# xswang/xflow

Measured on NVIDIA H100. Metric: training examples/sec, higher is better.
Workload: dtype f32

## Files before the change

xflow_b200/csrc/checkpoint.cu:

```cuda
#include <cuda_runtime.h>
#include <stddef.h>
#include <stdint.h>
#include <stdio.h>
#include <string.h>

#include <algorithm>
#include <string>
#include <vector>

#include "internal.h"

#define XF_ST_TILE 1024
#define XF_ST_VERSION 1u

struct XfStateHeader {
  char magic[4];
  uint32_t version;
  uint64_t header_bytes;
  uint64_t capacity;
  uint64_t cap_floor;
  uint64_t n_keys;
  uint32_t stride;
  uint32_t log2cap;
  uint32_t bshift;
  uint32_t lazy;
  int32_t latent_dim;
  int32_t optimizer;
  float alpha, beta, lambda1, lambda2, learning_rate;
  int32_t v_init;
  uint64_t seed;
  int32_t shard_index;
  int32_t num_shards;
  int32_t canonical_fm;
  uint32_t seq;
  uint64_t batches;
  uint64_t rejected_tokens;
  uint64_t admitted_keys;
  int32_t admit_mode;
  float admit_probability;
  uint32_t admit_threshold;
  uint32_t admit_log2_cells;
  uint32_t admit_hashes;
  uint32_t tracking;
  uint64_t admit_decay_batches;
  uint64_t admit_seed;
  uint64_t evict_max_idle_batches;
// ... 147 lines not shown
  if (lane == 0) atomicAdd(meta_out + 1, sum);
  if (blockIdx.x == 0 && threadIdx.x == 0) meta_out[0] = total;
}

__global__ void __launch_bounds__(256) xf_k_state_unpack(XfTableView t, uint32_t* __restrict__ stamp,
                                                         const uint8_t* __restrict__ in, uint64_t n, uint64_t first,
                                                         uint64_t chunk_slots, uint64_t tag,
                                                         unsigned long long* __restrict__ sum_out, int* __restrict__ bad) {
  const uint32_t q = t.stride / 16u;
  const uint64_t* meta = reinterpret_cast<const uint64_t*>(in + n * t.stride);
  const uint64_t items = n * q;
  unsigned long long sum = 0;
  for (uint64_t j = (uint64_t)blockIdx.x * blockDim.x + threadIdx.x; j < items; j += (uint64_t)gridDim.x * blockDim.x) {
    const uint64_t r = j / q;
    const uint32_t c16 = (uint32_t)(j - r * q);
    const uint64_t off = r * t.stride + 16u * c16;
    const uint4 v = *reinterpret_cast<const uint4*>(in + off);
    sum += xf_st_hash((uint64_t)v.x | ((uint64_t)v.y << 32), tag | off) +
           xf_st_hash((uint64_t)v.z | ((uint64_t)v.w << 32), tag | (off + 8));
    const uint64_t m = meta[r];
    if (c16 == 0) sum += xf_st_hash(m, tag | (n * t.stride + r * 8u));
    const uint64_t slot = (uint32_t)m;
    if (slot < first || slot >= first + chunk_slots || slot > t.mask) {
      if (c16 == 0) *bad = 1;
      continue;
    }
    *reinterpret_cast<uint4*>(xf_row(t, slot) + 16u * c16) = v;
    if (c16 == 0 && stamp != nullptr) stamp[slot] = (uint32_t)(m >> 32);
  }
  sum = xf_st_warp_sum(sum);
  if ((threadIdx.x & 31u) == 0) atomicAdd(sum_out, sum);
}

__global__ void __launch_bounds__(256) xf_k_state_sum(const uint64_t* __restrict__ p, uint64_t n_words, uint64_t off0,
                                                      unsigned long long* __restrict__ sum_out) {
  unsigned long long sum = 0;
  for (uint64_t i = (uint64_t)blockIdx.x * blockDim.x + threadIdx.x; i < n_words; i += (uint64_t)gridDim.x * blockDim.x)
    sum += xf_st_hash(p[i], off0 + i * 8u);
  sum = xf_st_warp_sum(sum);
  if ((threadIdx.x & 31u) == 0) atomicAdd(sum_out, sum);
}

static uint64_t xf_st_chunk_slots(uint32_t stride, uint64_t capacity) {
  uint64_t c = XF_ST_TILE;
  while (c * 2 <= capacity && c * 2 * (stride + 8ull) <= XF_ST_CHUNK_BYTES) c *= 2;
  return std::min(c, capacity);
}

struct XfStateIo {
  uint8_t* dev[2] = {nullptr, nullptr};
  uint8_t* pin[2] = {nullptr, nullptr};
  uint32_t* d_tiles[2] = {nullptr, nullptr};
  unsigned long long* d_small = nullptr;
  unsigned long long* h_small = nullptr;
  cudaStream_t copy = nullptr;
  cudaStream_t work = nullptr;
  cudaEvent_t done[2] = {nullptr, nullptr};
  cudaEvent_t copied[2] = {nullptr, nullptr};
  size_t bytes = 0;
  ~XfStateIo() {
    if (work) cudaStreamSynchronize(work);
    if (copy) cudaStreamSynchronize(copy);
    for (int b = 0; b < 2; ++b) {
      if (done[b]) cudaEventSynchronize(done[b]);
      if (dev[b]) cudaFree(dev[b]);
      if (pin[b]) cudaFreeHost(pin[b]);
// ... 95 lines not shown
    ++t->launches;
    XF_CUDA_TRY(cudaGetLastError());
    for (uint64_t j = 0; j < nf + 1; ++j) {
      if (j < nf) {
        const int b = (int)(j & 1);
        XF_CUDA_TRY(cudaMemcpyAsync(io.pin[b], t->d_filter + j * fc, fc, cudaMemcpyDeviceToHost, st));
        XF_CUDA_TRY(cudaEventRecord(io.copied[b], st));
      }
      if (j >= 1) {
        const int b = (int)((j - 1) & 1);
        XF_CUDA_TRY(cudaEventSynchronize(io.copied[b]));
        if (!xf_st_write(f, io.pin[b], fc)) { xf_set_error("write to %s failed", path); return XF_ERR_IO; }
      }
    }
    uint64_t s = 0;
    XF_CUDA_TRY(cudaMemcpyAsync(&s, io.d_small + 5, 8, cudaMemcpyDeviceToHost, st));
    XF_CUDA_TRY(cudaStreamSynchronize(st));
    if (!xf_st_write(f, &s, 8)) { xf_set_error("write to %s failed", path); return XF_ERR_IO; }
  }
  return XF_OK;
}

XF_DLL int xf_table_save_state(xf_table* t, const char* path, uint64_t user) {
  if (!t || !path) { xf_set_error("null argument"); return XF_ERR_ARG; }
  std::lock_guard<std::mutex> host_lock(t->host_mu);
  XF_CUDA_TRY(cudaSetDevice(t->cfg.device));
  XF_TRY(t->check_error());
  unsigned long long size = 0, counters[2] = {0ull, 0ull};
  XF_CUDA_TRY(cudaMemcpy(&size, t->d_size, sizeof(size), cudaMemcpyDeviceToHost));
  if (t->d_admit) XF_CUDA_TRY(cudaMemcpy(counters, t->d_admit, sizeof(counters), cudaMemcpyDeviceToHost));
  XfStateHeader h;
  memset(&h, 0, sizeof(h));
  memcpy(h.magic, "XFST", 4);
  h.version = XF_ST_VERSION;
  h.header_bytes = sizeof(h);
  h.capacity = t->view.mask + 1;
  h.cap_floor = t->cap_floor;
  h.n_keys = size;
  h.stride = t->view.stride;
  h.log2cap = t->view.log2cap;
  h.bshift = t->view.bshift;
  h.lazy = (uint32_t)t->view.lazy;
  h.latent_dim = t->cfg.latent_dim;
  h.optimizer = t->cfg.optimizer;
  h.alpha = t->cfg.alpha; h.beta = t->cfg.beta; h.lambda1 = t->cfg.lambda1; h.lambda2 = t->cfg.lambda2;
  h.learning_rate = t->cfg.learning_rate;
  h.v_init = t->view.v_init;
  h.seed = t->cfg.seed;
  h.shard_index = t->cfg.shard_index;
  h.num_shards = t->cfg.num_shards;
  h.canonical_fm = t->cfg.canonical_fm;
  h.seq = t->view.lazy ? t->seq : 0u;
  h.batches = t->admit_batches;
  h.rejected_tokens = counters[0];
  h.admitted_keys = counters[1];
  h.admit_mode = t->admit.mode;
  h.admit_probability = t->admit.probability;
  h.admit_threshold = t->admit.threshold;
  h.admit_log2_cells = t->admit.log2_cells;
  h.admit_hashes = t->admit.hashes;
  h.admit_decay_batches = t->admit.decay_batches;
  h.admit_seed = t->admit.seed;
  h.tracking = t->d_stamp != nullptr ? 1u : 0u;
  h.evict_max_idle_batches = t->evict.max_idle_batches;
  h.evict_max_keys = t->evict.max_keys;
  h.user = user;
  h.chunk_slots = xf_st_chunk_slots(h.stride, h.capacity);
// ... 130 lines not shown
    XF_CUDA_TRY(cudaEventRecord(io.done[b], st));
  }
  if (total != h.n_keys) { xf_set_error("state image %s: the rows section holds %llu rows, its header announces %llu", path, (unsigned long long)total, (unsigned long long)h.n_keys); return XF_ERR_IO; }
  uint64_t filter_stated = 0;
  if (h.filter_bytes) {
    const uint64_t fc = std::min<uint64_t>(h.filter_bytes, (uint64_t)1 << (63 - __builtin_clzll(io.bytes)));
    const uint64_t nf = h.filter_bytes / fc;
    for (uint64_t j = 0; j < nf; ++j) {
      const int b = (int)(j & 1);
      XF_CUDA_TRY(cudaEventSynchronize(io.copied[b]));
      if (!xf_st_read(f, io.pin[b], fc)) { xf_set_error("truncated state image %s", path); return XF_ERR_IO; }
      XF_CUDA_TRY(cudaMemcpyAsync(nw.filter + j * fc, io.pin[b], fc, cudaMemcpyHostToDevice, io.copy));
      XF_CUDA_TRY(cudaEventRecord(io.copied[b], io.copy));
    }
    if (!xf_st_read(f, &filter_stated, 8)) { xf_set_error("truncated state image %s", path); return XF_ERR_IO; }
    XF_CUDA_TRY(cudaEventRecord(io.done[0], io.copy));
    XF_CUDA_TRY(cudaStreamWaitEvent(st, io.done[0], 0));
    xf_k_state_sum<<<xf_grid_for(h.filter_bytes / 8, 256, 8), 256, 0, st>>>(reinterpret_cast<const uint64_t*>(nw.filter),
                                                                            h.filter_bytes / 8, 0ull, d_filter_sum);
    ++t->launches;
    XF_CUDA_TRY(cudaGetLastError());
  }
  XF_CUDA_TRY(cudaMemcpyAsync(io.h_small + 4, io.d_small + 4, 3 * sizeof(unsigned long long), cudaMemcpyDeviceToHost, st));
  XF_CUDA_TRY(cudaStreamSynchronize(st));
  XF_CUDA_TRY(cudaStreamSynchronize(io.copy));
  if (io.h_small[6] != 0 || io.h_small[4] != stated) {
    xf_set_error("state image %s: checksum mismatch in the rows section", path);
    return XF_ERR_IO;
  }
  if (h.filter_bytes && io.h_small[5] != filter_stated) {
    xf_set_error("state image %s: checksum mismatch in the admission filter section", path);
    return XF_ERR_IO;
  }
  return XF_OK;
}

XF_DLL int xf_table_load_state(xf_table* t, const char* path, uint64_t* user) {
  if (!t || !path) { xf_set_error("null argument"); return XF_ERR_ARG; }
  std::lock_guard<std::mutex> host_lock(t->host_mu);
  XF_CUDA_TRY(cudaSetDevice(t->cfg.device));
  XF_TRY(t->check_error());
  unsigned long long size = 0;
  XF_CUDA_TRY(cudaMemcpy(&size, t->d_size, sizeof(size), cudaMemcpyDeviceToHost));
  if (size != 0 || t->admit_batches != 0) {
    xf_set_error("xf_table_load_state needs a table that has never held state (this one has %llu keys and has run %llu "
                 "training batches)", size, (unsigned long long)t->admit_batches);
    return XF_ERR_STATE;
  }
  FILE* f = fopen(path, "rb");
  if (!f) { xf_set_error("cannot open %s", path); return XF_ERR_IO; }
  XfStateHeader h;
  memset(&h, 0, sizeof(h));
  const size_t got = fread(&h, 1, sizeof(h), f);
  int rc = XF_OK;
  if (xf_refuse_foreign(h.magic, got, path, "XFST") != XF_OK) {
    rc = XF_ERR_IO;
  } else if (got < 4 || memcmp(h.magic, "XFST", 4) != 0) {
    xf_set_error("%s is not a state image (no XFST magic)", path);
    rc = XF_ERR_IO;
  } else if (got != sizeof(h) || h.header_bytes != sizeof(h) || h.version != XF_ST_VERSION) {
    xf_set_error("state image %s: truncated header or unknown version %u", path, h.version);
    rc = XF_ERR_IO;
  } else if (h.header_checksum != xf_st_host_sum(&h, offsetof(XfStateHeader, header_checksum), 0) || !xf_st_header_sane(h)) {
    xf_set_error("state image %s: the header is damaged (checksum mismatch)", path);
    rc = XF_ERR_IO;
  }
  if (rc == XF_OK) rc = xf_st_match(t, h);
  XfStateNew nw;
  std::vector<uint64_t> ring;
  if (rc == XF_OK) rc = xf_st_load_body(t, f, path, h, nw, ring);
  fclose(f);
  if (rc != XF_OK) {
    cudaStreamSynchronize(t->stream);
    return rc;
  }
  if (h.ring_entries) XF_CUDA_TRY(cudaMemcpy(t->d_rows_by_seq, ring.data(), ring.size() * 8, cudaMemcpyHostToDevice));
  if (nw.admit) { t->d_admit = nw.admit; nw.admit = nullptr; }
  const unsigned long long counters[4] = {h.rejected_tokens, h.admitted_keys, 0ull, 0ull};
  XF_CUDA_TRY(cudaMemcpy(t->d_admit, counters, sizeof(counters), cudaMemcpyHostToDevice));
  const unsigned long long n_keys = h.n_keys;
  XF_CUDA_TRY(cudaMemcpy(t->d_size, &n_keys, sizeof(n_keys), cudaMemcpyHostToDevice));
  cudaFree(t->view.base);
  if (t->d_stamp) cudaFree(t->d_stamp);
  if (t->d_filter) cudaFree(t->d_filter);
  t->view.base = nw.base;
  t->view.mask = h.capacity - 1;
  t->view.log2cap = h.log2cap;
  t->view.bshift = h.bshift;
  t->d_stamp = nw.stamp;
  t->d_filter = nw.filter;
  nw.base = nullptr; nw.stamp = nullptr; nw.filter = nullptr;
  xf_admission_config_default(&t->admit);
  t->admit.mode = h.admit_mode;
  t->admit.probability = h.admit_probability;
  t->admit.threshold = h.admit_threshold;
  t->admit.log2_cells = h.admit_log2_cells;
  t->admit.hashes = h.admit_hashes;
  t->admit.decay_batches = h.admit_decay_batches;
  t->admit.seed = h.admit_seed;
  t->evict.max_idle_batches = h.tracking ? h.evict_max_idle_batches : 0;
// ... 20 lines not shown
```

xflow_b200/csrc/kernels.cu:

```cuda
#include <cuda_runtime.h>
#include <stdint.h>
#include <stdlib.h>

#include <mutex>
#include <set>
#include <utility>

#include "kernels.h"
#include "table.cuh"

__global__ void xf_k_fill(uint8_t* base, uint64_t cap, uint32_t stride, int lazy) {
  const uint64_t chunks_per_row = stride / 16;
  const uint64_t total = cap * chunks_per_row;
  for (uint64_t c = (uint64_t)blockIdx.x * blockDim.x + threadIdx.x; c < total;
       c += (uint64_t)gridDim.x * blockDim.x) {
    uint64_t r = c / chunks_per_row;
    uint32_t q = (uint32_t)(c % chunks_per_row);
    uint4 v = make_uint4(0, 0, 0, 0);
    if (q == 0) {
      v.x = 0xFFFFFFFFu; v.y = 0xFFFFFFFFu;
      if (!lazy) v.w = XF_NEG_ZERO_BITS;
    }
    *reinterpret_cast<uint4*>(base + r * stride + (uint64_t)q * 16) = v;
  }
// ... 28 lines not shown
    rows = (double)__ldg(rows_dev);
  }
  unsigned int live_acc = 0;
  const int K = t.K;
  const unsigned lane = threadIdx.x & 31u;
  const uint64_t gwarp = ((uint64_t)blockIdx.x * blockDim.x + threadIdx.x) >> 5;
  const uint64_t nwarps = ((uint64_t)gridDim.x * blockDim.x) >> 5;
  const int q = (int)(lane & (unsigned)(tps - 1));
  const int gi = (int)(lane / (unsigned)tps);
  const int ngroups = 32 / tps;
  const int leader = (int)(lane & ~(unsigned)(tps - 1));
  const unsigned group_mask = (tps == 32) ? 0xffffffffu : (((1u << tps) - 1u) << leader);
  const int nchunk = K / VEC;

  for (uint64_t base = gwarp * 32; base < n; base += nwarps * 32) {
    const uint64_t e_fwd = base + lane;
    const uint64_t e_i = (SLOTG && e_fwd < n) ? (n - 1 - e_fwd) : e_fwd;
    const uint64_t e_phys = (e_i < n_head) ? e_i : (uint64_t)extra_base + (e_i - n_head);
    const uint32_t s_lane = (e_fwd < n) ? __ldcs(slots + e_phys) : 0xFFFFFFFFu;
    unsigned pend = __ballot_sync(0xffffffffu, s_lane != 0xFFFFFFFFu);
    if (live_total != nullptr && lane == 0) live_acc += __popc(pend);

    while (pend) {
      const int cnt = __popc(pend);
      const unsigned src = (gi < cnt) ? __fns(pend, 0, gi + 1) : 0u;
      const uint32_t s = __shfl_sync(0xffffffffu, s_lane, (int)src);
      const uint64_t i = __shfl_sync(0xffffffffu, (unsigned long long)e_i, (int)src);
      const uint64_t i_phys = __shfl_sync(0xffffffffu, (unsigned long long)e_phys, (int)src);
      uint8_t* rowp = (gi < cnt) ? xf_row(t, s) : nullptr;
      pend = (cnt <= ngroups) ? 0u : (pend & ~((2u << __fns(pend, 0, ngroups)) - 1u));

      const bool lat = K > 0 && (part & 2) && rowp != nullptr;
      float* vp = lat ? xf_row_v(rowp) : nullptr;
      float* nvp = lat ? xf_row_nv(rowp, K) : nullptr;
      float* zvp = lat ? xf_row_zv(rowp, K) : nullptr;
      float v0[VEC], n0[VEC], z0[VEC];
#pragma unroll
      for (int e = 0; e < VEC; ++e) { v0[e] = 0.f; n0[e] = 0.f; z0[e] = 0.f; }
      const bool has0 = lat && q < nchunk;
      if (has0) {
        xf_ldv<VEC>(vp + q * VEC, v0);
        if (t.opt == XF_OPT_FTRL) { xf_ldv<VEC>(nvp + q * VEC, n0); xf_ldv<VEC>(zvp + q * VEC, z0); }
      }
      float p0[VEC];
#pragma unroll
      for (int e = 0; e < VEC; ++e) p0[e] = 0.f;
      if (SLOTG && v0_side != nullptr && has0) {
        const uint64_t tok = (i_phys < (uint64_t)extra_base) ? i_phys : (uint64_t)__ldg(slots + i_phys + extra_n);
        xf_ldv<VEC>(v0_side + tok * (uint64_t)K + q * VEC, p0);
      }
      float ca0[VEC];
#pragma unroll
      for (int e = 0; e < VEC; ++e) ca0[e] = 0.f;
      if (SLOTG && t.canon && has0) xf_ldv<VEC>(xf_row_ca(t, rowp) + q * VEC, ca0);
      double accL = 0.0, accA = 0.0;
      if (SLOTG && has0) {
        const double2 a = __ldcg(reinterpret_cast<const double2*>(xf_row_acc(rowp, K)));
        accL = a.x;
        accA = a.y;
      }
      XfHead h;
      h.key = 0; h.flags = 0; h.w = h.n = h.z = 0.f; h.g = 0.0;
      if (q == 0 && rowp != nullptr) h = xf_load_head(rowp);
      const uint64_t key = __shfl_sync(group_mask, (unsigned long long)h.key, leader);
      const uint32_t flags = __shfl_sync(group_mask, h.flags, leader);
      if (rowp == nullptr) continue;

      if (q == 0) {
// ... 45 lines not shown
              const float zero[VEC] = {};
              xf_stv<VEC>(xf_row_ca(t, rowp) + k, zero);
            } else {
#pragma unroll
              for (int e = 0; e < VEC; ++e) g[e] = xf_div_rows((float)(accA - (double)vp0[e] * accL), rows);
            }
          } else {
#pragma unroll
            for (int e = 0; e < VEC; ++e) g[e] = gv[i * (uint64_t)K + k + e];
          }
          if (t.opt == XF_OPT_FTRL) {
#pragma unroll
            for (int e = 0; e < VEC; ++e) xf_ftrl_coord(t, g[e], v[e], nn[e], zz[e]);
            xf_stv<VEC>(nvp + k, nn);
            xf_stv<VEC>(zvp + k, zz);
          } else {
#pragma unroll
            for (int e = 0; e < VEC; ++e) xf_sgd_coord(t, g[e], v[e]);
          }
          xf_stv<VEC>(vp + k, v);
        }
        if (SLOTG) {
          __syncwarp(group_mask);
          if (q == 0) *reinterpret_cast<double2*>(xf_row_acc(rowp, K)) = make_double2(0.0, 0.0);
        }
      }
    }
  }
  if (live_total != nullptr) {
    if (lane == 0 && live_acc) atomicAdd(&s_live, live_acc);
    __syncthreads();
    if (threadIdx.x == 0 && s_live) atomicAdd_system(live_total, (unsigned long long)s_live);
  }
}

template <bool INSERT>
__global__ void xf_k_probe(XfTableView t, const uint64_t* __restrict__ keys, uint64_t n,
                           uint32_t* __restrict__ slots, float* __restrict__ w_out, XfStampView sv) {
  for (uint64_t i = (uint64_t)blockIdx.x * blockDim.x + threadIdx.x; i < n;
       i += (uint64_t)gridDim.x * blockDim.x) {
    XfHead h;
    h.w = 0.f;
    int64_t s = xf_probe<INSERT, true>(t, keys[i], &h, &sv);
    slots[i] = s >= 0 ? (uint32_t)s : 0xFFFFFFFFu;
    if (w_out) {
      if (s >= 0) xf_apply_pending(t, h);
      w_out[i] = s >= 0 ? h.w : 0.f;
    }
  }
}

__global__ void xf_k_gather_v(XfTableView t, const uint32_t* __restrict__ slots, const uint64_t* __restrict__ keys,
                              uint64_t n, float* __restrict__ v_out) {
  const int K = t.K;
  const uint64_t total = n * (uint64_t)K;
  for (uint64_t x = (uint64_t)blockIdx.x * blockDim.x + threadIdx.x; x < total;
       x += (uint64_t)gridDim.x * blockDim.x) {
    const uint64_t i = x / K;
    const int k = (int)(x % K);
    const uint32_t s = slots[i];
    float v = 0.f;
    if (s != 0xFFFFFFFFu) {
      const uint8_t* rowp = xf_row(t, s);
      const uint32_t flags = __ldcg(reinterpret_cast<const uint32_t*>(rowp + XF_OFF_FLAGS));
      v = (flags & XF_FLAG_V_READY) ? __ldcg(reinterpret_cast<const float*>(rowp + 32) + k)
                                    : xf_v_init(t, keys[i], (uint32_t)k);
// ... 4 lines not shown

__global__ void xf_k_import(XfTableView t, const uint32_t* __restrict__ slots, uint64_t n,
                            const float* w, const float* nw, const float* zw, const float* v,
                            const float* nv, const float* zv) {
  const int K = t.K;
  const uint64_t per = (uint64_t)K + 1;
  const uint64_t total = n * per;
  for (uint64_t x = (uint64_t)blockIdx.x * blockDim.x + threadIdx.x; x < total;
       x += (uint64_t)gridDim.x * blockDim.x) {
    const uint64_t i = x / per;
    const int c = (int)(x % per);
    const uint32_t s = slots[i];
    if (s == 0xFFFFFFFFu) continue;
    uint8_t* rowp = xf_row(t, s);
    if (c == 0) {
      if (w) {
        if (t.lazy) {
          XfHead h;
          h.key = *reinterpret_cast<const uint64_t*>(rowp);
          h.w = w[i]; h.n = nw ? nw[i] : 0.f; h.z = zw ? zw[i] : 0.f; h.flags = 0u; h.g = 0.0;
          xf_lazy_store(t, rowp, h, true);
        } else {
          *reinterpret_cast<float2*>(rowp + XF_OFF_STATE) = make_float2(w[i], nw ? nw[i] : 0.f);
          *reinterpret_cast<float*>(rowp + XF_OFF_STATE + 8) = zw ? zw[i] : 0.f;
          *reinterpret_cast<unsigned long long*>(rowp + 8) = XF_NEG_ZERO_BITS64;
        }
      }
      if (v && K > 0) *reinterpret_cast<uint32_t*>(rowp + XF_OFF_FLAGS) = XF_FLAG_V_READY;
    } else if (v) {
      const int k = c - 1;
      xf_row_v(rowp)[k] = v[i * K + k];
      if (k == 0) *reinterpret_cast<double2*>(xf_row_acc(rowp, K)) = make_double2(0.0, 0.0);
      if (t.opt == XF_OPT_FTRL) {
        xf_row_nv(rowp, K)[k] = nv ? nv[i * K + k] : 0.f;
        xf_row_zv(rowp, K)[k] = zv ? zv[i * K + k] : 0.f;
      }
    }
  }
}

__global__ void xf_k_export(XfTableView t, const uint32_t* __restrict__ slots, const uint64_t* __restrict__ keys,
                            uint64_t n, float* w, float* nw, float* zw, float* v, float* nv, float* zv,
                            uint8_t* present) {
  const int K = t.K;
  const uint64_t per = (uint64_t)K + 1;
  const uint64_t total = n * per;
  for (uint64_t x = (uint64_t)blockIdx.x * blockDim.x + threadIdx.x; x < total;
       x += (uint64_t)gridDim.x * blockDim.x) {
    const uint64_t i = x / per;
    const int c = (int)(x % per);
    const uint32_t s = slots[i];
    const bool have = s != 0xFFFFFFFFu;
    const uint8_t* rowp = have ? xf_row(t, s) : nullptr;
    if (c == 0) {
      XfHead h;
      h.w = h.n = h.z = 0.f;
      if (have) {
        h = xf_load_head(rowp);
        xf_apply_pending(t, h);
      }
      if (present) present[i] = have ? 1 : 0;
      if (w) w[i] = h.w;
      if (nw) nw[i] = h.n;
      if (zw) zw[i] = h.z;
    } else if (v) {
      const int k = c - 1;
      float vv = 0.f, nn = 0.f, zz = 0.f;
      if (have) {
        const uint32_t flags = __ldcg(reinterpret_cast<const uint32_t*>(rowp + XF_OFF_FLAGS));
        if (flags & XF_FLAG_V_READY) {
          vv = __ldcg(reinterpret_cast<const float*>(rowp + 32) + k);
          if (t.opt == XF_OPT_FTRL) {
            nn = __ldcg(xf_row_nv(const_cast<uint8_t*>(rowp), K) + k);
            zz = __ldcg(xf_row_zv(const_cast<uint8_t*>(rowp), K) + k);
          }
        } else {
          vv = xf_v_init(t, keys[i], (uint32_t)k);
        }
      }
      v[i * K + k] = vv;
      if (nv) nv[i * K + k] = nn;
      if (zv) zv[i * K + k] = zz;
    }
  }
}

__global__ void xf_k_rehash(XfTableView src, XfTableView dst, XfKeep keep, const uint32_t* __restrict__ src_stamp,
                            uint32_t* __restrict__ dst_stamp) {
  const uint64_t cap = src.mask + 1;
  const uint32_t chunks = src.stride / 16;
  for (uint64_t r = (uint64_t)blockIdx.x * blockDim.x + threadIdx.x; r < cap;
       r += (uint64_t)gridDim.x * blockDim.x) {
    const uint8_t* srow = xf_row(src, r);
    uint4 a = *reinterpret_cast<const uint4*>(srow);
    uint64_t key = (uint64_t)a.x | ((uint64_t)a.y << 32);
    if (key == XF_EMPTY_KEY) continue;
    const uint32_t stamp = src_stamp != nullptr ? src_stamp[r] : 0u;
    if (src_stamp != nullptr && !xf_keeps(keep, stamp, key)) continue;
    XfHead h;
    int64_t s = xf_probe<true>(dst, key, &h);
    if (s < 0) continue;
    uint8_t* drow = xf_row(dst, (uint64_t)s);
    *reinterpret_cast<uint2*>(drow + 8) = make_uint2(a.z, a.w);
    for (uint32_t c = 1; c < chunks; ++c)
      *reinterpret_cast<uint4*>(drow + 16 * c) = *reinterpret_cast<const uint4*>(srow + 16 * c);
    if (dst_stamp != nullptr) dst_stamp[s] = stamp;
  }
// ... 33 lines not shown
    int dev = 0;
    cudaGetDevice(&dev);
    std::lock_guard<std::mutex> lock(mu);
    if (done.insert({dev, kernel}).second)
      cudaFuncSetAttribute(kernel, cudaFuncAttributeMaxDynamicSharedMemorySize, (int)smem);
  }
  const int per_sm = (int)(227 * 1024 / (smem + 1024));
  return xf_grid_for(work_items, block, per_sm < 8 ? per_sm : 8);
}

int xf_vec_for(int K) { return K <= 0 ? 1 : (K % 4 == 0 ? 4 : (K % 2 == 0 ? 2 : 1)); }
int xf_tps_for(int K) {
  if (K <= 0) return 1;
  int chunks = K / xf_vec_for(K);
  int tps = 1;
  while (tps < chunks && tps < 32) tps <<= 1;
  return tps;
}

void xf_launch_fill(const XfTableView& t, cudaStream_t st) {
  uint64_t cap = t.mask + 1;
  uint64_t total = cap * (t.stride / 16);
  xf_k_fill<<<xf_grid_for(total, 256, 16), 256, 0, st>>>(t.base, cap, t.stride, t.lazy);
}

template <bool SLOTG, bool STAMP = false>
static void xf_launch_update_t(const XfTableView& t, const uint32_t* slots, uint64_t n, double rows,
                               const float* gw, const float* gv, int part, unsigned long long* live_total,
                               cudaStream_t st, const uint32_t* n_dev = nullptr, const uint32_t* rows_dev = nullptr,
                               uint32_t extra_base = 0, uint32_t extra_n = 0, const float* v0_side = nullptr,
                               XfStampView sv = XfStampView{nullptr, 0u}) {
  const int tps = xf_tps_for(t.K);
  const int grid = xf_grid_for(n * (uint64_t)tps, 256, 8);
#define XF_UPD_ARGS t, slots, n, tps, rows, gw, gv, part, live_total, n_dev, rows_dev, extra_base, extra_n, v0_side, sv
  switch (xf_vec_for(t.K)) {
    case 4: xf_k_update<4, SLOTG, STAMP><<<grid, 256, 0, st>>>(XF_UPD_ARGS); break;
    case 2: xf_k_update<2, SLOTG, STAMP><<<grid, 256, 0, st>>>(XF_UPD_ARGS); break;
    default: xf_k_update<1, SLOTG, STAMP><<<grid, 256, 0, st>>>(XF_UPD_ARGS); break;
  }
#undef XF_UPD_ARGS
}

void xf_launch_update_touched_dev(const XfTableView& t, const uint32_t* touched, uint64_t work_bound,
                                  const uint32_t* n_dev, const uint32_t* rows_dev, uint32_t extra_base,
                                  uint32_t extra_n, const float* v0_side, unsigned long long* unique_total,
                                  cudaStream_t st) {
  xf_launch_update_t<true>(t, touched, work_bound + extra_n, 1.0, nullptr, nullptr, 3, unique_total, st, n_dev, rows_dev,
                           extra_base, extra_n, v0_side);
}

__global__ void xf_k_flush_pending(XfTableView t) {
  const uint64_t cap = t.mask + 1;
  for (uint64_t r = (uint64_t)blockIdx.x * blockDim.x + threadIdx.x; r < cap; r += (uint64_t)gridDim.x * blockDim.x) {
    uint8_t* rowp = xf_row(t, r);
    XfHead h = xf_load_head(rowp);
    if (h.key == XF_EMPTY_KEY || !xf_lazy_has_pending(h)) continue;
    xf_apply_pending(t, h);
    xf_lazy_store(t, rowp, h);
  }
}
void xf_launch_flush_pending(const XfTableView& t, cudaStream_t st) {
  xf_k_flush_pending<<<xf_grid_for(t.mask + 1, 256, 8), 256, 0, st>>>(t);
}

void xf_launch_update_touched(const XfTableView& t, const uint32_t* touched, uint64_t nnz, double rows,
                              unsigned long long* unique_total, const XfStampView& sv, cudaStream_t st) {
// ... 51 lines not shown
```

xflow_b200/csrc/table.cuh:

```cuda
#pragma once
#include <cuda_runtime.h>
#include <stdint.h>

#define XF_EMPTY_KEY 0xFFFFFFFFFFFFFFFFull
#define XF_FLAG_V_READY 1u
#define XF_NEG_ZERO_BITS 0x80000000u
#define XF_NEG_ZERO_BITS64 0x8000000000000000ull
#define XF_MAX_PROBE 8192

enum { XF_OPT_FTRL = 0, XF_OPT_SGD = 1 };
enum { XF_INIT_DEFAULT = 0, XF_INIT_COUNTER = 1, XF_INIT_ZERO = 3 };

struct XfTableView {
  uint8_t* base;
  uint64_t mask;
  uint32_t log2cap;
  uint32_t bshift;
  uint32_t stride;
  int K;
  int opt;
  int v_init;
  float v_const;
  uint64_t seed;
  float alpha, beta, lambda1, lambda2, learning_rate;
// ... 17 lines not shown
  unsigned long long* rej_n;
  uint64_t* rej_keys;
  unsigned long long* admitted;
};
struct XfKeep {
  uint32_t cutoff;
  int bounded;
  uint32_t s_star;
  uint64_t k_star;
};
struct XfStampView {
  uint32_t* stamp;
  uint32_t now;
};
struct XfWeightView {
  const float* e;
  const unsigned long long* W;
};
__host__ __device__ __forceinline__ bool xf_keeps(const XfKeep& k, uint32_t stamp, uint64_t key) {
  return stamp >= k.cutoff && (!k.bounded || stamp > k.s_star || (stamp == k.s_star && key <= k.k_star));
}
#define XF_TAG_LOCKED 0xFFFFFFFFu
#define XF_FIX_MAX_SHIFT 27
#define XF_TAG_MASK 0xFFFFull

__host__ __device__ inline int xf_fix_shift(uint64_t nnz) {
  int bits = 0;
  while (bits < 64 && (nnz >> bits) != 0ull) ++bits;
  const int s = 47 - bits;
  return s > XF_FIX_MAX_SHIFT ? XF_FIX_MAX_SHIFT : (s < 0 ? 0 : s);
}

__host__ __device__ inline uint32_t xf_acc_off(int K) { return (32u + 4u * (uint32_t)K + 15u) & ~15u; }
__host__ __device__ inline uint32_t xf_ca_off(int K, int opt) {
  return xf_acc_off(K) + 16u + ((opt == XF_OPT_FTRL) ? 8u * (uint32_t)K : 0u);
}
__host__ __device__ inline uint32_t xf_row_stride(int K, int opt, int canon = 0) {
  if (K <= 0) return 32u;
  uint32_t bytes = xf_ca_off(K, opt) + (canon ? 4u * (uint32_t)K : 0u);
  return (bytes + 31u) & ~31u;
}

#ifdef __CUDACC__

__device__ __forceinline__ uint64_t xf_probe_slot(const XfTableView& t, uint64_t key, uint32_t i) {
  const uint64_t m = key * 0x9E3779B97F4A7C15ull;
  const uint32_t bs = t.bshift;
  const uint64_t hb = m >> (64 - (t.log2cap - bs));
  const uint32_t b1 = (1u << bs) - 1u;
  const uint32_t j0 = (uint32_t)(m >> 9) & b1;
  const uint32_t k = i >> bs;
  const uint32_t j = (k == 0) ? ((j0 + i) & b1) : (i & b1);
  return (((hb + k) << bs) | j) & t.mask;
}
__device__ __forceinline__ uint64_t xf_home_slot(const XfTableView& t, uint64_t key) { return xf_probe_slot(t, key, 0); }

__host__ __device__ __forceinline__ uint64_t xf_splitmix64(uint64_t x) {
  x += 0x9E3779B97F4A7C15ull;
  x = (x ^ (x >> 30)) * 0xBF58476D1CE4E5B9ull;
  x = (x ^ (x >> 27)) * 0x94D049BB133111EBull;
  return x ^ (x >> 31);
}
__host__ __device__ __forceinline__ uint64_t xf_admit_cell(uint64_t key, uint64_t seed, uint32_t j, uint32_t log2_cells) {
  return xf_splitmix64(key ^ xf_splitmix64(seed + (uint64_t)(j + 1) * 0x9E3779B97F4A7C15ull)) >> (64 - log2_cells);
}
__device__ __forceinline__ bool xf_admit(const XfAdmitView& a, uint64_t key) {
  if (a.mode == XF_ADM_POISSON) return (uint32_t)(xf_splitmix64(key ^ a.batch_mix) >> 40) < a.p24;
  if (a.mode != XF_ADM_BLOOM) return false;
  uint32_t m = 255u;
  for (uint32_t j = 0; j < a.hashes; ++j) m = min(m, (uint32_t)__ldcg(a.cells + xf_admit_cell(key, a.seed, j, a.log2_cells)));
  return m >= a.threshold;
}
__device__ __forceinline__ void xf_admit_append(const XfAdmitView& a, bool r0, uint64_t k0, bool r1, uint64_t k1) {
  const unsigned m0 = __ballot_sync(0xffffffffu, r0), m1 = __ballot_sync(0xffffffffu, r1);
// ... 18 lines not shown
  if (a.rej_keys && r) a.rej_keys[base + __popc(m & ((1u << lane) - 1u))] = k;
}

__device__ __forceinline__ float xf_counter_normal(uint64_t key, uint32_t k, uint64_t seed) {
  uint64_t base = xf_splitmix64(key ^ xf_splitmix64(seed + 0x632BE59BD9B4E019ull * (uint64_t)(k + 1)));
  uint32_t sum = 0;
#pragma unroll
  for (int r = 0; r < 3; ++r) {
    uint64_t x = xf_splitmix64(base + (uint64_t)r);
    sum += (uint32_t)(x & 0xFFFF) + (uint32_t)((x >> 16) & 0xFFFF) + (uint32_t)((x >> 32) & 0xFFFF) +
           (uint32_t)((x >> 48) & 0xFFFF);
  }
  float u = __fmul_rn((float)((int32_t)sum - 6 * 65535), 1.0f / 65536.0f);
  return __fmul_rn(u, 1e-2f);
}
__device__ __forceinline__ float xf_v_init(const XfTableView& t, uint64_t key, uint32_t k) {
  if (t.v_init == XF_INIT_COUNTER) return xf_counter_normal(key, k, t.seed);
  if (t.v_init == XF_INIT_ZERO) return 0.0f;
  return t.v_const;
}
__device__ __forceinline__ float4 xf_v_init_piece(const XfTableView& t, uint64_t key, uint32_t q) {
  return make_float4(xf_v_init(t, key, 4 * q), xf_v_init(t, key, 4 * q + 1), xf_v_init(t, key, 4 * q + 2),
                     xf_v_init(t, key, 4 * q + 3));
}

__device__ __forceinline__ uint8_t* xf_row(const XfTableView& t, uint64_t slot) {
  return t.base + slot * (uint64_t)t.stride;
}
__device__ __forceinline__ double* xf_row_g(uint8_t* row) { return reinterpret_cast<double*>(row + 8); }
#define XF_OFF_STATE 16
#define XF_OFF_FLAGS 28
__device__ __forceinline__ float* xf_row_v(uint8_t* row) { return reinterpret_cast<float*>(row + 32); }
__device__ __forceinline__ double* xf_row_acc(uint8_t* row, int K) { return reinterpret_cast<double*>(row + xf_acc_off(K)); }
__device__ __forceinline__ float* xf_row_nv(uint8_t* row, int K) { return reinterpret_cast<float*>(row + xf_acc_off(K) + 16); }
__device__ __forceinline__ float* xf_row_zv(uint8_t* row, int K) { return xf_row_nv(row, K) + K; }
__device__ __forceinline__ float* xf_row_ca(const XfTableView& t, uint8_t* row) { return reinterpret_cast<float*>(row + xf_ca_off(t.K, t.opt)); }

struct XfHead {
  uint64_t key;
  uint32_t flags;
  float w, n, z;
  double g;
};

__device__ __forceinline__ void xf_ld32_cg(const void* p, uint64_t& q0, uint64_t& q1, uint64_t& q2, uint64_t& q3) {
  asm volatile("ld.global.cg.v2.u64 {%0,%1}, [%4];\n\tld.global.cg.v2.u64 {%2,%3}, [%4+16];"
               : "=l"(q0), "=l"(q1), "=l"(q2), "=l"(q3) : "l"(p));
}
__device__ __forceinline__ void xf_ld32_ca(const void* p, uint64_t& q0, uint64_t& q1, uint64_t& q2, uint64_t& q3) {
  asm volatile("ld.global.ca.v2.u64 {%0,%1}, [%4];\n\tld.global.ca.v2.u64 {%2,%3}, [%4+16];"
               : "=l"(q0), "=l"(q1), "=l"(q2), "=l"(q3) : "l"(p));
}
__device__ __forceinline__ void xf_ld32_pair(const uint8_t* mine, uint64_t& q0, uint64_t& q1, uint64_t& q2, uint64_t& q3) {
  const uint32_t odd = threadIdx.x & 1u;
  const uint8_t* other = (const uint8_t*)__shfl_xor_sync(0xffffffffu, (unsigned long long)mine, 1);
  const uint8_t* r0 = odd ? other : mine;
  const uint8_t* r1 = odd ? mine : other;
  uint64_t x0 = 0, x1 = 0, y0 = 0, y1 = 0;
  asm volatile("{\n .reg .pred p0, p1;\n setp.ne.u64 p0, %4, 0;\n setp.ne.u64 p1, %5, 0;\n"
               " @p0 ld.global.cg.v2.u64 {%0,%1}, [%6];\n @p1 ld.global.cg.v2.u64 {%2,%3}, [%7];\n}"
               : "+l"(x0), "+l"(x1), "+l"(y0), "+l"(y1)
               : "l"(r0), "l"(r1), "l"(r0 + 16 * odd), "l"(r1 + 16 * odd));
  const uint64_t m0 = odd ? y0 : x0, m1 = odd ? y1 : x1;
  const uint64_t t0 = __shfl_xor_sync(0xffffffffu, odd ? x0 : y0, 1);
  const uint64_t t1 = __shfl_xor_sync(0xffffffffu, odd ? x1 : y1, 1);
  q0 = odd ? t0 : m0; q1 = odd ? t1 : m1;
  q2 = odd ? m0 : t0; q3 = odd ? m1 : t1;
}
__device__ __forceinline__ void xf_st32(void* p, uint64_t q0, uint64_t q1, uint64_t q2, uint64_t q3) {
// ... 326 lines not shown
```

Measured before the change: 92.83 million.

## Align FTRL latent state to 32-byte lines and add line-wise update kernel

Moves the FTRL n/z latent arrays to a 32-byte-aligned offset when this fits inside the existing row stride, so for K=16 the second half of each 256-byte row starts at byte 128. Adds a specialised update kernel for K=16 FTRL that has groups of 8 lanes load each row as two 128-byte coalesced vectors, exchange fields with shuffles, and write full lines back. The aim is fewer and wider memory transactions per row update. Checkpoints gain a version field and a realign kernel that converts old packed images on load, which adds format complexity.

```diff
diff --git a/xflow_b200/csrc/checkpoint.cu b/xflow_b200/csrc/checkpoint.cu
--- a/xflow_b200/csrc/checkpoint.cu
+++ b/xflow_b200/csrc/checkpoint.cu
@@ -11,7 +11,11 @@
 #include "internal.h"
 
 #define XF_ST_TILE 1024
-#define XF_ST_VERSION 1u
+#define XF_ST_VERSION_PACKED 1u
+#define XF_ST_VERSION_ALIGNED 2u
+static uint32_t xf_st_version(const XfTableView& v, int canonical_fm) {
+  return xf_nv_off(v.K, v.opt, canonical_fm) != xf_acc_off(v.K) + 16u ? XF_ST_VERSION_ALIGNED : XF_ST_VERSION_PACKED;
+}
 
 struct XfStateHeader {
   char magic[4];
@@ -225,6 +229,18 @@
   if ((threadIdx.x & 31u) == 0) atomicAdd(sum_out, sum);
 }
 
+__global__ void xf_k_state_realign(XfTableView t, uint32_t from, uint32_t to, uint32_t words) {
+  const uint64_t cap = t.mask + 1;
+  for (uint64_t r = (uint64_t)blockIdx.x * blockDim.x + threadIdx.x; r < cap; r += (uint64_t)gridDim.x * blockDim.x) {
+    uint8_t* row = xf_row(t, r);
+    if (*reinterpret_cast<const uint64_t*>(row) == XF_EMPTY_KEY) continue;
+    uint32_t* src = reinterpret_cast<uint32_t*>(row + from);
+    uint32_t* dst = reinterpret_cast<uint32_t*>(row + to);
+    for (uint32_t i = words; i-- > 0;) dst[i] = src[i];
+    for (uint32_t i = 0; i < (to - from) / 4u; ++i) src[i] = 0u;
+  }
+}
+
 __global__ void __launch_bounds__(256) xf_k_state_sum(const uint64_t* __restrict__ p, uint64_t n_words, uint64_t off0,
                                                       unsigned long long* __restrict__ sum_out) {
   unsigned long long sum = 0;
@@ -386,7 +402,7 @@
   XfStateHeader h;
   memset(&h, 0, sizeof(h));
   memcpy(h.magic, "XFST", 4);
-  h.version = XF_ST_VERSION;
+  h.version = xf_st_version(t->view, t->cfg.canonical_fm);
   h.header_bytes = sizeof(h);
   h.capacity = t->view.mask + 1;
   h.cap_floor = t->cap_floor;
@@ -583,6 +599,14 @@
     xf_set_error("state image %s: checksum mismatch in the admission filter section", path);
     return XF_ERR_IO;
   }
+  const uint32_t packed = xf_acc_off(h.latent_dim) + 16u, aligned = xf_nv_off(h.latent_dim, h.optimizer, h.canonical_fm);
+  if (h.version == XF_ST_VERSION_PACKED && aligned != packed) {
+    const uint32_t words = 2u * (uint32_t)h.latent_dim + (h.canonical_fm ? (uint32_t)h.latent_dim : 0u);
+    xf_k_state_realign<<<xf_grid_for(h.capacity, 256, 8), 256, 0, st>>>(v, packed, aligned, words);
+    ++t->launches;
+    XF_CUDA_TRY(cudaGetLastError());
+    XF_CUDA_TRY(cudaStreamSynchronize(st));
+  }
   return XF_OK;
 }
 
@@ -609,7 +633,8 @@
   } else if (got < 4 || memcmp(h.magic, "XFST", 4) != 0) {
     xf_set_error("%s is not a state image (no XFST magic)", path);
     rc = XF_ERR_IO;
-  } else if (got != sizeof(h) || h.header_bytes != sizeof(h) || h.version != XF_ST_VERSION) {
+  } else if (got != sizeof(h) || h.header_bytes != sizeof(h) ||
+             (h.version != XF_ST_VERSION_PACKED && h.version != XF_ST_VERSION_ALIGNED)) {
     xf_set_error("state image %s: truncated header or unknown version %u", path, h.version);
     rc = XF_ERR_IO;
   } else if (h.header_checksum != xf_st_host_sum(&h, offsetof(XfStateHeader, header_checksum), 0) || !xf_st_header_sane(h)) {
@@ -617,6 +642,11 @@
     rc = XF_ERR_IO;
   }
   if (rc == XF_OK) rc = xf_st_match(t, h);
+  if (rc == XF_OK && h.version == XF_ST_VERSION_ALIGNED && xf_st_version(t->view, t->cfg.canonical_fm) != h.version) {
+    xf_set_error("state image %s: version 2 holds aligned FTRL latent rows, which this table (latent_dim %d, optimizer %d) "
+                 "does not have", path, t->cfg.latent_dim, t->cfg.optimizer);
+    rc = XF_ERR_IO;
+  }
   XfStateNew nw;
   std::vector<uint64_t> ring;
   if (rc == XF_OK) rc = xf_st_load_body(t, f, path, h, nw, ring);
diff --git a/xflow_b200/csrc/kernels.cu b/xflow_b200/csrc/kernels.cu
--- a/xflow_b200/csrc/kernels.cu
+++ b/xflow_b200/csrc/kernels.cu
@@ -84,8 +84,8 @@
 
       const bool lat = K > 0 && (part & 2) && rowp != nullptr;
       float* vp = lat ? xf_row_v(rowp) : nullptr;
-      float* nvp = lat ? xf_row_nv(rowp, K) : nullptr;
-      float* zvp = lat ? xf_row_zv(rowp, K) : nullptr;
+      float* nvp = lat ? xf_row_nv(t, rowp) : nullptr;
+      float* zvp = lat ? xf_row_zv(t, rowp) : nullptr;
       float v0[VEC], n0[VEC], z0[VEC];
 #pragma unroll
       for (int e = 0; e < VEC; ++e) { v0[e] = 0.f; n0[e] = 0.f; z0[e] = 0.f; }
@@ -197,6 +197,110 @@
     __syncthreads();
     if (threadIdx.x == 0 && s_live) atomicAdd_system(live_total, (unsigned long long)s_live);
   }
+}
+
+template <bool STAMP>
+__global__ void __launch_bounds__(256)
+xf_k_update_lines(XfTableView t, const uint32_t* __restrict__ slots, uint64_t n, double rows,
+                  unsigned long long* __restrict__ live_total, XfStampView sv) {
+  __shared__ unsigned int s_live;
+  if (threadIdx.x == 0) s_live = 0;
+  __syncthreads();
+  unsigned int live_acc = 0;
+  const unsigned lane = threadIdx.x & 31u;
+  const uint64_t gwarp = ((uint64_t)blockIdx.x * blockDim.x + threadIdx.x) >> 5;
+  const uint64_t nwarps = ((uint64_t)gridDim.x * blockDim.x) >> 5;
+  const unsigned p = lane & 7u, gi = lane >> 3;
+  const int leader = (int)(lane & ~7u);
+  const unsigned group_mask = 0xFFu << leader;
+  const unsigned c = p & 3u, hh = p >> 2;
+  const int k0 = (int)(4u * c + 2u * hh);
+
+  for (uint64_t base = gwarp * 32; base < n; base += nwarps * 32) {
+    const uint64_t e_fwd = base + lane;
+    const uint64_t e_i = e_fwd < n ? n - 1 - e_fwd : e_fwd;
+    const uint32_t s_lane = (e_fwd < n) ? __ldcs(slots + e_i) : 0xFFFFFFFFu;
+    unsigned pend = __ballot_sync(0xffffffffu, s_lane != 0xFFFFFFFFu);
+    if (live_total != nullptr && lane == 0) live_acc += __popc(pend);
+
+    while (pend) {
+      const int cnt = __popc(pend);
+      const unsigned src = ((int)gi < cnt) ? __fns(pend, 0, gi + 1) : 0u;
+      const uint32_t s = __shfl_sync(0xffffffffu, s_lane, (int)src);
+      uint8_t* rowp = ((int)gi < cnt) ? xf_row(t, s) : nullptr;
+      pend = (cnt <= 4) ? 0u : (pend & ~((2u << __fns(pend, 0, 4)) - 1u));
+
+      uint4 a0 = make_uint4(0u, 0u, 0u, 0u), a1 = make_uint4(0u, 0u, 0u, 0u);
+      if (rowp != nullptr) {
+        a0 = __ldcg(reinterpret_cast<const uint4*>(rowp) + p);
+        a1 = __ldcg(reinterpret_cast<const uint4*>(rowp + 128) + p);
+      }
+      const uint32_t key_lo = __shfl_sync(0xffffffffu, a0.x, leader), key_hi = __shfl_sync(0xffffffffu, a0.y, leader);
+      const uint32_t flags = __shfl_sync(0xffffffffu, a0.w, leader + 1);
+      const uint32_t g_lo = __shfl_xor_sync(0xffffffffu, a0.z, 1), g_hi = __shfl_xor_sync(0xffffffffu, a0.w, 1);
+      const uint32_t L_lo = __shfl_sync(0xffffffffu, a0.x, leader + 6), L_hi = __shfl_sync(0xffffffffu, a0.y, leader + 6);
+      const uint32_t A_lo = __shfl_sync(0xffffffffu, a0.z, leader + 6), A_hi = __shfl_sync(0xffffffffu, a0.w, leader + 6);
+      const int vsrc = leader + 2 + (int)c;
+      const uint32_t vx = __shfl_sync(0xffffffffu, a0.x, vsrc), vy = __shfl_sync(0xffffffffu, a0.y, vsrc);
+      const uint32_t vz = __shfl_sync(0xffffffffu, a0.z, vsrc), vw = __shfl_sync(0xffffffffu, a0.w, vsrc);
+      const uint32_t x0 = __shfl_xor_sync(0xffffffffu, hh ? a1.x : a1.z, 4);
+      const uint32_t x1 = __shfl_xor_sync(0xffffffffu, hh ? a1.y : a1.w, 4);
+      if (rowp == nullptr) continue;
+
+      const uint64_t key = (uint64_t)key_lo | ((uint64_t)key_hi << 32);
+      const double accL = __hiloint2double((int)L_hi, (int)L_lo), accA = __hiloint2double((int)A_hi, (int)A_lo);
+      float v[2], nn[2], zz[2];
+      v[0] = __uint_as_float(hh ? vz : vx);
+      v[1] = __uint_as_float(hh ? vw : vy);
+      nn[0] = __uint_as_float(hh ? x0 : a1.x);
+      nn[1] = __uint_as_float(hh ? x1 : a1.y);
+      zz[0] = __uint_as_float(hh ? a1.z : x0);
+      zz[1] = __uint_as_float(hh ? a1.w : x1);
+      if (!(flags & XF_FLAG_V_READY)) {
+#pragma unroll
+        for (int e = 0; e < 2; ++e) { v[e] = xf_v_init(t, key, (uint32_t)(k0 + e)); nn[e] = 0.f; zz[e] = 0.f; }
+      }
+#pragma unroll
+      for (int e = 0; e < 2; ++e) {
+        const float g = xf_div_rows((float)(accA - (double)v[e] * accL), rows);
+        xf_ftrl_coord(t, g, v[e], nn[e], zz[e]);
+      }
+      uint4 o0 = a0;
+      if (p == 0u) {
+        o0.z = 0u;
+        o0.w = XF_NEG_ZERO_BITS;
+        if (STAMP) sv.stamp[s] = sv.now;
+      } else if (p == 1u) {
+        float w = __uint_as_float(a0.x), nw = __uint_as_float(a0.y), zw = __uint_as_float(a0.z);
+        const float g = xf_div_rows((float)__hiloint2double((int)g_hi, (int)g_lo), rows);
+        xf_ftrl_coord(t, g, w, nw, zw);
+        o0 = make_uint4(__float_as_uint(w), __float_as_uint(nw), __float_as_uint(zw), a0.w | XF_FLAG_V_READY);
+      } else if (p == 6u) {
+        o0 = make_uint4(0u, 0u, 0u, 0u);
+      }
+      const int pc = (int)(p - 2u) & 3;
+      const uint32_t u0 = __shfl_sync(group_mask, __float_as_uint(v[0]), leader + pc);
+      const uint32_t u1 = __shfl_sync(group_mask, __float_as_uint(v[1]), leader + pc);
+      const uint32_t u2 = __shfl_sync(group_mask, __float_as_uint(v[0]), leader + 4 + pc);
+      const uint32_t u3 = __shfl_sync(group_mask, __float_as_uint(v[1]), leader + 4 + pc);
+      const uint32_t y0 = __shfl_xor_sync(group_mask, __float_as_uint(hh ? nn[0] : zz[0]), 4);
+      const uint32_t y1 = __shfl_xor_sync(group_mask, __float_as_uint(hh ? nn[1] : zz[1]), 4);
+      if (p >= 2u && p < 6u) o0 = make_uint4(u0, u1, u2, u3);
+      const uint4 o1 = hh ? make_uint4(y0, y1, __float_as_uint(zz[0]), __float_as_uint(zz[1]))
+                          : make_uint4(__float_as_uint(nn[0]), __float_as_uint(nn[1]), y0, y1);
+      reinterpret_cast<uint4*>(rowp)[p] = o0;
+      reinterpret_cast<uint4*>(rowp + 128)[p] = o1;
+    }
+  }
+  if (live_total != nullptr) {
+    if (lane == 0 && live_acc) atomicAdd(&s_live, live_acc);
+    __syncthreads();
+    if (threadIdx.x == 0 && s_live) atomicAdd_system(live_total, (unsigned long long)s_live);
+  }
+}
+static bool xf_upd_lines(const XfTableView& t) {
+  return t.K == 16 && t.opt == XF_OPT_FTRL && !t.canon && !t.lazy && t.stride == 256u &&
+         xf_acc_off(16) + 16u <= 128u && xf_nv_off(16, XF_OPT_FTRL, 0) == 128u;
 }
 
 template <bool INSERT>
@@ -267,8 +371,8 @@
       xf_row_v(rowp)[k] = v[i * K + k];
       if (k == 0) *reinterpret_cast<double2*>(xf_row_acc(rowp, K)) = make_double2(0.0, 0.0);
       if (t.opt == XF_OPT_FTRL) {
-        xf_row_nv(rowp, K)[k] = nv ? nv[i * K + k] : 0.f;
-        xf_row_zv(rowp, K)[k] = zv ? zv[i * K + k] : 0.f;
+        xf_row_nv(t, rowp)[k] = nv ? nv[i * K + k] : 0.f;
+        xf_row_zv(t, rowp)[k] = zv ? zv[i * K + k] : 0.f;
       }
     }
   }
@@ -306,8 +410,8 @@
         if (flags & XF_FLAG_V_READY) {
           vv = __ldcg(reinterpret_cast<const float*>(rowp + 32) + k);
           if (t.opt == XF_OPT_FTRL) {
-            nn = __ldcg(xf_row_nv(const_cast<uint8_t*>(rowp), K) + k);
-            zz = __ldcg(xf_row_zv(const_cast<uint8_t*>(rowp), K) + k);
+            nn = __ldcg(xf_row_nv(t, const_cast<uint8_t*>(rowp)) + k);
+            zz = __ldcg(xf_row_zv(t, const_cast<uint8_t*>(rowp)) + k);
           }
         } else {
           vv = xf_v_init(t, keys[i], (uint32_t)k);
@@ -407,6 +511,10 @@
                                XfStampView sv = XfStampView{nullptr, 0u}) {
   const int tps = xf_tps_for(t.K);
   const int grid = xf_grid_for(n * (uint64_t)tps, 256, 8);
+  if (SLOTG && n_dev == nullptr && v0_side == nullptr && part == 3 && xf_upd_lines(t)) {
+    xf_k_update_lines<STAMP><<<xf_grid_for(n * 8ull, 256, 8), 256, 0, st>>>(t, slots, n, rows, live_total, sv);
+    return;
+  }
 #define XF_UPD_ARGS t, slots, n, tps, rows, gw, gv, part, live_total, n_dev, rows_dev, extra_base, extra_n, v0_side, sv
   switch (xf_vec_for(t.K)) {
     case 4: xf_k_update<4, SLOTG, STAMP><<<grid, 256, 0, st>>>(XF_UPD_ARGS); break;
diff --git a/xflow_b200/csrc/table.cuh b/xflow_b200/csrc/table.cuh
--- a/xflow_b200/csrc/table.cuh
+++ b/xflow_b200/csrc/table.cuh
@@ -73,14 +73,22 @@
 }
 
 __host__ __device__ inline uint32_t xf_acc_off(int K) { return (32u + 4u * (uint32_t)K + 15u) & ~15u; }
-__host__ __device__ inline uint32_t xf_ca_off(int K, int opt) {
-  return xf_acc_off(K) + 16u + ((opt == XF_OPT_FTRL) ? 8u * (uint32_t)K : 0u);
-}
-__host__ __device__ inline uint32_t xf_row_stride(int K, int opt, int canon = 0) {
+__host__ __device__ inline uint32_t xf_packed_stride(int K, int opt, int canon) {
   if (K <= 0) return 32u;
-  uint32_t bytes = xf_ca_off(K, opt) + (canon ? 4u * (uint32_t)K : 0u);
+  const uint32_t bytes = xf_acc_off(K) + 16u + ((opt == XF_OPT_FTRL) ? 8u * (uint32_t)K : 0u) + (canon ? 4u * (uint32_t)K : 0u);
   return (bytes + 31u) & ~31u;
 }
+__host__ __device__ inline uint32_t xf_nv_off(int K, int opt, int canon = 0) {
+  const uint32_t packed = xf_acc_off(K) + 16u;
+  if (opt != XF_OPT_FTRL || K <= 0) return packed;
+  const uint32_t aligned = (packed + 31u) & ~31u;
+  const uint32_t bytes = aligned + 8u * (uint32_t)K + (canon ? 4u * (uint32_t)K : 0u);
+  return ((bytes + 31u) & ~31u) == xf_packed_stride(K, opt, canon) ? aligned : packed;
+}
+__host__ __device__ inline uint32_t xf_ca_off(int K, int opt, int canon = 0) {
+  return xf_nv_off(K, opt, canon) + ((opt == XF_OPT_FTRL) ? 8u * (uint32_t)K : 0u);
+}
+__host__ __device__ inline uint32_t xf_row_stride(int K, int opt, int canon = 0) { return xf_packed_stride(K, opt, canon); }
 
 #ifdef __CUDACC__
 
@@ -165,9 +173,13 @@
 #define XF_OFF_FLAGS 28
 __device__ __forceinline__ float* xf_row_v(uint8_t* row) { return reinterpret_cast<float*>(row + 32); }
 __device__ __forceinline__ double* xf_row_acc(uint8_t* row, int K) { return reinterpret_cast<double*>(row + xf_acc_off(K)); }
-__device__ __forceinline__ float* xf_row_nv(uint8_t* row, int K) { return reinterpret_cast<float*>(row + xf_acc_off(K) + 16); }
-__device__ __forceinline__ float* xf_row_zv(uint8_t* row, int K) { return xf_row_nv(row, K) + K; }
-__device__ __forceinline__ float* xf_row_ca(const XfTableView& t, uint8_t* row) { return reinterpret_cast<float*>(row + xf_ca_off(t.K, t.opt)); }
+__device__ __forceinline__ float* xf_row_nv(const XfTableView& t, uint8_t* row) {
+  return reinterpret_cast<float*>(row + xf_nv_off(t.K, t.opt, t.canon));
+}
+__device__ __forceinline__ float* xf_row_zv(const XfTableView& t, uint8_t* row) { return xf_row_nv(t, row) + t.K; }
+__device__ __forceinline__ float* xf_row_ca(const XfTableView& t, uint8_t* row) {
+  return reinterpret_cast<float*>(row + xf_ca_off(t.K, t.opt, t.canon));
+}
 
 struct XfHead {
   uint64_t key;
```

Result: no change. 92.94 million, median of 6 (+0.1%).
